# sp-uhh/buddy

Measured on AMD Instinct MI355X. Metric: diffusion steps/sec (4 s@16 kHz utterance, blind Euler-Heun DPS, order 1, 10 operator updates/step), higher is better.
Workload: dtype f32 (GEMM operands -- Winograd-domain and 1x1 / NIN -- as two-term f16 splits, 2^-22, fp32 accumulation)

## Files before the change

buddy_amd/_lib.py:

```python
from __future__ import annotations

import ctypes as C
import os

_HERE = os.path.dirname(os.path.abspath(__file__))
LIB_PATH = os.path.join(_HERE, "libbuddy_hip.so")


class BuddyHipError(RuntimeError):
    pass


_lib = None

_f32p = C.c_void_p
_SIGS = {
    "buddy_last_error": (C.c_char_p, []),
    "buddy_version": (C.c_int, []),
    "buddy_ncsnpp_param_count": (C.c_int, [C.c_int, C.POINTER(C.c_int), C.c_int, C.c_int, C.POINTER(C.c_longlong)]),
    "buddy_ncsnpp_create": (C.c_int, [_f32p, C.c_longlong, C.c_int, C.POINTER(C.c_int), C.c_int, C.c_int, C.c_int, C.c_int,
                                      C.POINTER(C.c_void_p)]),
    "buddy_ncsnpp_param_count_attn": (C.c_int, [C.c_int, C.POINTER(C.c_int), C.c_int, C.c_int, C.c_int, C.POINTER(C.c_longlong)]),
    "buddy_ncsnpp_create_attn": (C.c_int, [_f32p, C.c_longlong, C.c_int, C.POINTER(C.c_int), C.c_int, C.c_int, C.c_int, C.c_int, C.c_int,
                                           C.POINTER(C.c_void_p)]),
# ... 116 lines not shown
    "buddy_blindop_degrade": (C.c_int, [C.c_void_p, _f32p, _f32p, C.c_void_p]),
    "buddy_blindop_time_rir": (C.c_int, [C.c_void_p, _f32p, C.c_void_p]),
    "buddy_blindop_design_filter": (C.c_int, [C.c_void_p, _f32p, C.c_void_p]),
    "buddy_blindop_apply_stft": (C.c_int, [C.c_void_p, _f32p, _f32p, C.c_void_p]),
    "buddy_blindop_degrade_vjp": (C.c_int, [C.c_void_p, _f32p, _f32p, _f32p, _f32p, C.c_void_p]),
    "buddy_blindop_time_rir_vjp": (C.c_int, [C.c_void_p, _f32p, _f32p, C.c_void_p]),
    "buddy_blindop_update_H_vjp": (C.c_int, [C.c_void_p, _f32p, _f32p, _f32p, _f32p, C.c_void_p]),
    "buddy_blindop_stft": (C.c_int, [C.c_void_p, _f32p, C.c_int, _f32p, C.c_void_p]),
    "buddy_blindop_stft_adjoint": (C.c_int, [C.c_void_p, _f32p, C.c_int, _f32p, C.c_void_p]),
    "buddy_blindop_stft_loss": (C.c_int, [C.c_void_p, _f32p, _f32p, C.c_int, C.c_float, _f32p, _f32p, _f32p, C.c_void_p]),
    "buddy_blindop_set_compression": (C.c_int, [C.c_void_p, C.c_float]),
    "buddy_blindop_set_loss_norm": (C.c_int, [C.c_void_p, C.c_int]),
    "buddy_blindop_set_loss": (C.c_int, [C.c_void_p, C.c_int, C.c_int, C.c_int, C.c_float]),
    "buddy_blindop_set_freq_weights": (C.c_int, [C.c_void_p, C.c_int, _f32p]),
    "buddy_blindop_lengths": (C.c_int, [C.c_void_p, C.POINTER(C.c_int), C.POINTER(C.c_int), C.POINTER(C.c_int), C.POINTER(C.c_int)]),
    "buddy_blindop_minphase": (C.c_int, [C.c_void_p, _f32p, _f32p, C.c_void_p]),
    "buddy_blindop_project": (C.c_int, [C.c_void_p, C.c_void_p]),
    "buddy_blindop_get_adam": (C.c_int, [C.c_void_p, _f32p, _f32p, _f32p, _f32p, _f32p, _f32p, C.POINTER(C.c_int), C.c_void_p]),
    "buddy_blindop_rec_loss_grad": (C.c_int, [C.c_void_p, _f32p, C.c_float, _f32p, _f32p, C.c_void_p]),
    "buddy_blindop_fir_loss_grad": (C.c_int, [C.c_void_p, _f32p, _f32p, C.c_longlong, C.c_int, C.c_float, _f32p, _f32p, C.c_void_p]),
    "buddy_blindop_param_grads": (C.c_int, [C.c_void_p, _f32p, _f32p, C.c_float, C.c_float, C.c_float, _f32p, _f32p, _f32p, _f32p, C.c_void_p]),
    "buddy_blindop_optimize": (C.c_int, [C.c_void_p, _f32p, _f32p, C.c_float, C.c_int, C.c_float, C.c_float, C.c_float, C.c_float, C.c_float,
                                         C.c_float, C.c_void_p]),
    "buddy_fir": (C.c_int, [_f32p, _f32p, C.c_longlong, _f32p, C.c_int, C.c_int, C.c_int, C.c_int, C.c_void_p]),
}
EXPORTED = sorted(_SIGS)


def load():
    global _lib
# ... 43 lines not shown
```

buddy_amd/csrc/capi.hip:

```cpp
#include "../../include/buddy_hip.h"
#include "common.h"
#include "net.h"

#include <cstring>

using namespace buddy;

namespace buddy {
void launch_axpby_rows(const float* x, const float* y, const float* a, const float* c, float* out, int B, int L, hipStream_t st);
void launch_row_moments(const float* x, double* out, int B, int L, hipStream_t st);
void launch_perturb(const float* x, const float* eps, float scale, float* out, long long n, hipStream_t st);
void launch_dps_update(const float* x_hat, const float* x_den, const float* lh, const float* lh_scale_b, const float* den_scale_b, const float* base, const float* d_prev,
                       float t, float dt, float w_prev, float w_cur, float* out, float* d_out, float* x_den_out, int B, int L, hipStream_t st);
void launch_row_scale(const float* x, float* out, int B, int L, int mode, float p0, float p1, hipStream_t st);
void launch_fill_rows4(float* out, int B, float v0, float v1, float v2, float v3, hipStream_t st);
void launch_mfma_ubench(const float* seed, float* out, int blocks, int iters, unsigned long long* clk, hipStream_t st);
void launch_mfma_ubench_bf16(const float* seed, float* out, int blocks, int iters, unsigned long long* clk, hipStream_t st);
int launch_hbm_ubench(const void* src, void* dst, long long bytes, int mode, int nt, int blocks, hipStream_t st);
void launch_fir(const float* x, const float* h, long long h_stride, float* y, int B, int L, int M, int adjoint, hipStream_t st);
}

static int finish() {
  hipError_t e = hipGetLastError();
  if (e != hipSuccess) { set_error(std::string("kernel launch: ") + hipGetErrorString(e)); return BUDDY_ERR_HIP; }
// ... 658 lines not shown
int buddy_blindop_time_rir_vjp(void* h, const float* g_rir, float* g_H, void* stream) { BOP_CHECK(h); if (!g_rir || !g_H) { set_error("null"); return BUDDY_ERR_ARG; } return blindop_time_rir_vjp((BlindOp*)h, g_rir, g_H, (hipStream_t)stream); }
int buddy_blindop_update_H_vjp(void* h, const float* g_H, float* g_decay, float* g_weights, float* g_phases, void* stream) {
  BOP_CHECK(h); if (!g_H) { set_error("null"); return BUDDY_ERR_ARG; } return blindop_update_H_vjp((BlindOp*)h, g_H, g_decay, g_weights, g_phases, (hipStream_t)stream);
}
int buddy_blindop_stft(void* h, const float* x, int len, float* X, void* stream) { BOP_CHECK(h); if (!x || !X) { set_error("null"); return BUDDY_ERR_ARG; } return blindop_stft_len((BlindOp*)h, x, len, X, (hipStream_t)stream); }
int buddy_blindop_stft_adjoint(void* h, const float* G, int len, float* g_x, void* stream) { BOP_CHECK(h); if (!G || !g_x) { set_error("null"); return BUDDY_ERR_ARG; } return blindop_stft_len_adj((BlindOp*)h, G, len, g_x, (hipStream_t)stream); }
int buddy_blindop_stft_loss(void* h, const float* a, const float* b, int len, float weight, float* loss, float* g_a, float* g_b, void* stream) {
  BOP_CHECK(h); if (!a || !b || !loss) { set_error("null"); return BUDDY_ERR_ARG; } return blindop_stft_loss((BlindOp*)h, a, b, len, weight, loss, g_a, g_b, (hipStream_t)stream);
}
int buddy_blindop_set_compression(void* h, float comp) { BOP_CHECK(h); return blindop_set_compression((BlindOp*)h, comp); }
int buddy_blindop_set_loss_norm(void* h, int mode) { BOP_CHECK(h); return blindop_set_loss_norm((BlindOp*)h, mode); }
int buddy_blindop_set_loss(void* h, int slot, int kind, int freq_weighting, float compression) {
  BOP_CHECK(h); return blindop_set_loss((BlindOp*)h, slot, kind, freq_weighting, compression);
}
int buddy_blindop_set_freq_weights(void* h, int freq_weighting, const float* w) { BOP_CHECK(h); return blindop_set_freq_weights((BlindOp*)h, freq_weighting, w); }
int buddy_blindop_lengths(void* h, int* L, int* Lr, int* T, int* Td) { BOP_CHECK(h); return blindop_lengths((BlindOp*)h, L, Lr, T, Td); }
int buddy_blindop_minphase(void* h, const float* hin, float* out, void* stream) { BOP_CHECK(h); if (!hin || !out) { set_error("null"); return BUDDY_ERR_ARG; } return blindop_minphase((BlindOp*)h, hin, out, (hipStream_t)stream); }
int buddy_blindop_project(void* h, void* stream) { BOP_CHECK(h); return blindop_project((BlindOp*)h, (hipStream_t)stream); }
int buddy_blindop_get_adam(void* h, float* m_decay, float* v_decay, float* m_weights, float* v_weights, float* m_phases, float* v_phases, int* step,
                           void* stream) {
  BOP_CHECK(h); return blindop_get_adam((BlindOp*)h, m_decay, v_decay, m_weights, v_weights, m_phases, v_phases, step, (hipStream_t)stream);
}
int buddy_blindop_rec_loss_grad(void* h, const float* x_den, float weight, float* loss, float* g_x, void* stream) {
  BOP_CHECK(h); if (!x_den || !loss) { set_error("null"); return BUDDY_ERR_ARG; }
  return blindop_rec_loss_grad((BlindOp*)h, x_den, weight, loss, g_x, (hipStream_t)stream);
}
int buddy_blindop_fir_loss_grad(void* h, const float* x_den, const float* rir, long long rir_stride, int M, float weight, float* loss, float* g_x,
                                void* stream) {
  BOP_CHECK(h); if (!x_den || !rir || !loss || M < 1) { set_error("bad arguments"); return BUDDY_ERR_ARG; }
  return blindop_fir_loss_grad((BlindOp*)h, x_den, rir, rir_stride, M, weight, loss, g_x, (hipStream_t)stream);
// ... 14 lines not shown
```

buddy_amd/csrc/net.h:

```cpp
#pragma once
#include <hip/hip_runtime.h>
#include <string>

namespace buddy {

struct NetCfg { int nf; int ch_mult[8]; int nlev; int nrb; int n_fft; int hop; int attn_mask; };
struct Net;

void set_error(const std::string& s);
const char* last_error();
long long param_count(const NetCfg& c);
int net_create(const float* host_params, long long n, const NetCfg& cfg, Net** out);
void net_destroy(Net* N);
int net_replica(Net* src, Net** out);
int net_weight_bytes(Net* N, long long* params, long long* packed, long long* lazy, int* lazy_forms);
int net_set_option(Net* N, const char* key, int value);
int net_get_option(Net* N, const char* key, int* value);
int net_set_gemm(Net* N, int mode);
int net_set_attention(Net* N, int mode);
int net_set_fir(Net* N, int fir);
int net_reserve(Net* N, int B, int L, int with_vjp, long long* bytes);
int net_forward(Net* N, const float* x, const float* cnoise, const float* cin_b, const float* cskip_b, const float* cout_b, float* y, int B, int L,
                int save, hipStream_t st);
int net_vjp(Net* N, const float* cot, float* gx, hipStream_t st);
// ... 23 lines not shown
int blindop_apply_stft(BlindOp* o, const float* x, float* X_ref, hipStream_t st);
int blindop_minphase(BlindOp* o, const float* h, float* out, hipStream_t st);
int blindop_project(BlindOp* o, hipStream_t st);
int blindop_get_adam(BlindOp* o, float* m_decay, float* v_decay, float* m_wts, float* v_wts, float* m_phases, float* v_phases, int* step, hipStream_t st);
int blindop_degrade_vjp(BlindOp* o, const float* x, const float* g_y, float* g_x, float* g_H_ref, hipStream_t st);
int blindop_time_rir_vjp(BlindOp* o, const float* g_rir, float* g_H_ref, hipStream_t st);
int blindop_update_H_vjp(BlindOp* o, const float* g_H_ref, float* g_decay, float* g_wts, float* g_phases_ref, hipStream_t st);
int blindop_stft_len(BlindOp* o, const float* x, int len, float* X_ref, hipStream_t st);
int blindop_stft_len_adj(BlindOp* o, const float* G_ref, int len, float* g_x, hipStream_t st);
int blindop_stft_loss(BlindOp* o, const float* a, const float* b, int len, float weight, float* loss, float* g_a, float* g_b, hipStream_t st);
int blindop_set_compression(BlindOp* o, float comp);
int blindop_set_loss_norm(BlindOp* o, int mode);
int blindop_set_loss(BlindOp* o, int slot, int kind, int freq_weighting, float comp);
int blindop_set_freq_weights(BlindOp* o, int freq_weighting, const float* w);
int blindop_lengths(BlindOp* o, int* L, int* Lr, int* T, int* Td);
int blindop_rec_loss_grad(BlindOp* o, const float* x_den, float weight, float* loss, float* g_x, hipStream_t st);
int blindop_fir_loss_grad(BlindOp* o, const float* x_den, const float* rir, long long rir_stride, int M, float weight, float* loss, float* g_x,
                          hipStream_t st);
int blindop_param_grads(BlindOp* o, const float* x_den, const float* noise, float t_op, float w_rec, float w_reg, float* g_decay, float* g_wts,
                        float* g_phases_ref, float* losses, hipStream_t st);
int blindop_optimize(BlindOp* o, const float* x_den, const float* noise, float t_op, int n_iters, float w_rec, float w_reg, float lr, float b1,
                     float b2, float wd, hipStream_t st);

}
```

buddy_amd/csrc/operator.hip:

```cpp
#include "common.h"
#include "net.h"

#include <cmath>
#include <cstring>
#include <vector>

namespace buddy {

#define HIPCHK(x) do { hipError_t e_ = (x); if (e_ != hipSuccess) { set_error(std::string(#x) + ": " + hipGetErrorString(e_)); return BUDDY_ERR_HIP; } } while (0)

namespace {
constexpr int FB = 513, LDSP = 1028, NFFT = 1024, WIN = 512, HOP = 128;
constexpr int N2 = 25856, F1 = 101, F2 = 256;
constexpr double PI = 3.14159265358979323846;

constexpr int FT = 4;
__global__ __launch_bounds__(256) void fir_kernel_sb(const float* X, long long xs, const float* H, float* Y, int U, int T, int Nf) {
  const int TG = (T + FT - 1) / FT;
  const long long total = (long long)U * TG * FB;
  for (long long i = (long long)blockIdx.x * 256 + threadIdx.x; i < total; i += (long long)gridDim.x * 256) {
    const int f = (int)(i % FB); const int t0 = (int)((i / FB) % TG) * FT; const int u = (int)(i / ((long long)FB * TG));
    const float2* Xu = reinterpret_cast<const float2*>(X + (long long)u * xs) + f;
    const float2* Hu = reinterpret_cast<const float2*>(H + (long long)u * Nf * LDSP) + f;
    auto ldx = [&](int tt) { return (tt >= 0 && tt < T) ? Xu[(long long)tt * (LDSP / 2)] : make_float2(0.f, 0.f); };
// ... 202 lines not shown
}

__device__ __forceinline__ float2 compress(float2 x, float p) {
  const float r = sqrtf(x.x * x.x + x.y * x.y);
  if (r == 0.f) return make_float2(powf(1e-8f, p), 0.f);
  const float rho = powf(r + 1e-8f, p) / r;
  return make_float2(x.x * rho, x.y * rho);
}
__global__ __launch_bounds__(256) void compress_kernel(const float* X, float* Xc, long long rows, float p) {
  const long long total = rows * FB;
  for (long long i = (long long)blockIdx.x * 256 + threadIdx.x; i < total; i += (long long)gridDim.x * 256) {
    const long long r = i / FB; const int f = (int)(i % FB);
    reinterpret_cast<float2*>(Xc + r * LDSP)[f] = compress(reinterpret_cast<const float2*>(X + r * LDSP)[f], p);
  }
}
struct LossJob { const float* Rc; const float* Xh; float* G; double* partial; int T; float kappa; int blocks; };
struct LossJobs { LossJob j[2]; };
__global__ __launch_bounds__(256) void comp_loss_kernel(LossJobs jobs, float p) {
  __shared__ double red[256];
  const bool second = (int)blockIdx.x >= jobs.j[0].blocks;
  const LossJob& jb = jobs.j[second ? 1 : 0];
  const float* Rc = jb.Rc; const float* Xh = jb.Xh; float* G = jb.G;
  const int T = jb.T, nblk = jb.blocks, bx = (int)blockIdx.x - (second ? jobs.j[0].blocks : 0);
  const float kappa = jb.kappa;
  const int u = blockIdx.y;
  const long long total = (long long)T * FB;
  double acc = 0.0;
  for (long long i = (long long)bx * 256 + threadIdx.x; i < total; i += (long long)nblk * 256) {
    const long long t = i / FB; const int f = (int)(i % FB);
    const long long row = ((long long)u * T + t) * LDSP;
    const float2 x = reinterpret_cast<const float2*>(Xh + row)[f];
    const float2 rc = Rc ? reinterpret_cast<const float2*>(Rc + row)[f] : compress(reinterpret_cast<const float2*>(G + row)[f], p);
    const float r = sqrtf(x.x * x.x + x.y * x.y);
    float2 g = make_float2(0.f, 0.f);
    float2 xc;
    if (r == 0.f) {
      xc = make_float2(powf(1e-8f, p), 0.f);
    } else {
      const float ir = 1.f / r, re = r + 1e-8f;
      const float cr = x.x * ir, ci = x.y * ir;
      const float rho = powf(re, p);
      xc = make_float2(rho * cr, rho * ci);
      const float dr = xc.x - rc.x, di = xc.y - rc.y;
      const float a = dr * cr + di * ci;
      const float b = dr * ci - di * cr;
      const float gr = 2.f * kappa * a * p * (rho / re);
      const float gt = -2.f * kappa * rho * b * ir;
      g = make_float2(gr * cr - gt * ci, gr * ci + gt * cr);
    }
    const float dr = xc.x - rc.x, di = xc.y - rc.y;
    acc += (double)(dr * dr + di * di);
    if (G) reinterpret_cast<float2*>(G + row)[f] = g;
  }
  red[threadIdx.x] = acc;
  __syncthreads();
  for (int off = 128; off > 0; off >>= 1) { if (threadIdx.x < off) red[threadIdx.x] += red[threadIdx.x + off]; __syncthreads(); }
  if (threadIdx.x == 0) jb.partial[(long long)u * nblk + bx] = red[0];
}
__global__ void loss_finalize_kernel(const double* partial, int nblk, float kappa, float* loss, int accumulate) {
  const int u = blockIdx.x;
  if (threadIdx.x != 0) return;
  double s = 0.0;
  for (int i = 0; i < nblk; ++i) s += partial[(long long)u * nblk + i];
  const float v = (float)(s * (double)kappa);
  loss[u] = accumulate ? loss[u] + v : v;
}
// ... 614 lines not shown
  const bool ok = row < (second ? jobs.j[1].rows : jobs.j[0].rows);
  const float2* f = reinterpret_cast<const float2*>(in + (ok ? row : 0) * LDSP);
  float2 v[16];
#pragma unroll
  for (int a = 0; a < 16; ++a) {
    const int k = 64 * a + r;
    float2 x = make_float2(0.f, 0.f);
    if (ok && k <= 512) { x = f[k]; if (cf && k != 0 && k != 512) { x.x *= 2.f; x.y *= 2.f; } }
    v[a] = x;
  }
  fft1024_core<1>(v, S[w], tw, r);
  if (!ok) return;
#pragma unroll
  for (int c1 = 0; c1 < 8; ++c1) { const int n = r + 64 * c1; frames[row * WIN + n] = fac * win[n] * v[c1].x; }
}

__global__ __launch_bounds__(256) void adam_kernel(float* p, const float* g, float* m, float* v, long long n, float lr, float b1, float b2, float eps,
                                                   float wd, float bc1, float bc2_sqrt, const int* step_dev, const float2* bc_tab) {
  if (step_dev) { const float2 bc = bc_tab[*step_dev]; bc1 = bc.x; bc2_sqrt = bc.y; }
  for (long long i = (long long)blockIdx.x * 256 + threadIdx.x; i < n; i += (long long)gridDim.x * 256) {
    float gi = g[i];
    if (wd != 0.f) gi += wd * p[i];
    const float mi = m[i] + (gi - m[i]) * (1.f - b1);
    const float vi = v[i] * b2 + (1.f - b2) * gi * gi;
    m[i] = mi; v[i] = vi;
    const float denom = sqrtf(vi) / bc2_sqrt + eps;
    p[i] = p[i] - (lr / bc1) * (mi / denom);
  }
}
__global__ void set_scalar_kernel(float* dst, float v) { *dst = v; }
// ... 120 lines not shown
struct BlindOp {
  BlindOpCfg c;
  int U = 0, L = 0, T = 0, Td = 0, Lr = 0, Lh = 0, Lm = 0, E = 0, NB = 0, K = 0, Nf = 0;
  hipStream_t st = nullptr;
  std::vector<void*> allocs;
  float *ones = nullptr, *env_T = nullptr, *env_d = nullptr, *env_c = nullptr;
  float norm = 1.f;
  int *idx = nullptr, *fge = nullptr; float *frac = nullptr, *corr = nullptr, *dpm = nullptr;
  float2 *w101 = nullptr, *w256 = nullptr, *twN = nullptr, *w1024r = nullptr, *w64t = nullptr; float* win = nullptr;
  float *decay = nullptr, *wts = nullptr, *phi = nullptr;
  float *m_d = nullptr, *v_d = nullptr, *m_w = nullptr, *v_w = nullptr, *m_p = nullptr, *v_p = nullptr;
  int adam_step = 0;
  static constexpr int MAXSTEP = 65536;
  int* d_step = nullptr; float* d_scal = nullptr; float2* bc_tab = nullptr; float tab_b1 = -1.f, tab_b2 = -1.f;
  float *xden_buf = nullptr, *noise_buf = nullptr; int noise_iters = 0;
  hipStream_t cap_stream = nullptr; hipGraphExec_t gexec = nullptr; int g_iters = -1; float g_hp[7] = {0, 0, 0, 0, 0, 0, 0};
  float *H = nullptr, *Yc = nullptr, *Xdelta = nullptr;
  float *frames = nullptr, *X1 = nullptr, *X2 = nullptr, *X3 = nullptr, *Ybuf = nullptr, *sig1 = nullptr, *sig2 = nullptr;
  float *frames_b = nullptr, *X2_b = nullptr, *X3_b = nullptr, *Ybuf_b = nullptr; double* partial_b = nullptr;
  struct LossDesc { int kind; int fw; float comp; };
  static constexpr int NSLOT = 4, NFW = 5;
  LossDesc slot[NSLOT] = {{0, 0, 0.667f}, {0, 0, 0.667f}, {0, 0, 0.667f}, {0, 0, 0.667f}};
  float* wtab = nullptr; unsigned wtab_set = 1u;
  float *Ytd = nullptr, *Yc1 = nullptr;
  bool fused_loop = false;
  bool big_lds = false;
  float *A = nullptr, *Apre = nullptr, *logdm = nullptr, *dmv = nullptr, *gdm = nullptr, *Fin = nullptr, *GFin = nullptr, *GH = nullptr;
  float *gphi = nullptr, *gdecay = nullptr, *gw = nullptr, *hm = nullptr, *gh0 = nullptr;
  float2 *c1 = nullptr, *c2 = nullptr, *Hf = nullptr;
  float *Mabs = nullptr, *phim = nullptr, *gM = nullptr;
  double* partial = nullptr; float* losses = nullptr;
// ... 129 lines not shown
  static bool is_comp(const LossDesc& d) { return d.kind <= LK_COMP_MEAN; }
  static bool legacy(const LossDesc& d) { return is_comp(d) && d.fw == 0; }
  static bool same_target(const LossDesc& a, const LossDesc& b) {
    if (is_td(a) || is_td(b)) return is_td(a) && is_td(b);
    if (!is_spec(a) || !is_spec(b) || a.fw != b.fw) return false;
    if (is_comp(a) || is_comp(b)) return is_comp(a) && is_comp(b) && a.comp == b.comp;
    return a.kind == b.kind;
  }
  const float* wrow(const LossDesc& d) const { return d.fw ? wtab + (size_t)d.fw * FB : nullptr; }
  const float* target(int s) const { return is_td(slot[s]) ? Ytd : (s == 1 && !same_target(slot[0], slot[1]) ? Yc1 : Yc); }
  void spec_target(int s, const float* X, float* R, long long rows) {
    const LossDesc& d = slot[s];
    if (legacy(d)) hipLaunchKernelGGL(compress_kernel, dim3(gridf(rows * FB)), dim3(256), 0, st, X, R, rows, d.comp);
    else hipLaunchKernelGGL(spec_target_kernel, dim3(gridf(rows * FB)), dim3(256), 0, st, X, R, rows, d.kind, wrow(d), d.comp);
  }
  static constexpr int LOSS_BLK = 64, LOSS_BLK_B = 32;
  void comp_loss2(int s0, const float* Rc0, const float* Xh0, float* G0, int T0, float w0, float* out0, int s1, const float* Rc1, const float* Xh1, float* G1,
                  int T1, float w1, float* out1, bool two) {
    const LossDesc& d0 = slot[s0];
    const LossDesc& d1 = slot[two ? s1 : s0];
    auto kap = [&](const LossDesc& d, float w, int Tn) { return d.kind == LK_COMP_SUMMEAN ? w / (float)Tn : (d.kind == LK_COMP_MEAN ? w / ((float)Tn * (float)FB) : w); };
    const float k0 = kap(d0, w0, T0), k1 = two ? kap(d1, w1, T1) : 0.f;
    const unsigned grid = LOSS_BLK + (two ? LOSS_BLK_B : 0);
    if (legacy(d0) && (!two || (legacy(d1) && d1.comp == d0.comp))) {
      LossJobs jobs; std::memset(&jobs, 0, sizeof(jobs));
      jobs.j[0] = LossJob{Rc0, Xh0, G0, partial, T0, k0, LOSS_BLK};
      if (two) jobs.j[1] = LossJob{Rc1, Xh1, G1, partial_b, T1, k1, LOSS_BLK_B};
      hipLaunchKernelGGL(comp_loss_kernel, dim3(grid, U), dim3(256), 0, st, jobs, d0.comp);
    } else {
      SpecJobs jobs; std::memset(&jobs, 0, sizeof(jobs));
      jobs.j[0] = SpecJob{Rc0, Xh0, G0, partial, wrow(d0), T0, k0, d0.comp, d0.kind, LOSS_BLK};
      if (two) jobs.j[1] = SpecJob{Rc1, Xh1, G1, partial_b, wrow(d1), T1, k1, d1.comp, d1.kind, LOSS_BLK_B};
      hipLaunchKernelGGL(spec_loss_kernel, dim3(grid, U), dim3(256), 0, st, jobs);
    }
    if (!fused_loop) {
      hipLaunchKernelGGL(loss_finalize_kernel, dim3(U), dim3(32), 0, st, (const double*)partial, LOSS_BLK, k0, out0, 0);
      if (two) hipLaunchKernelGGL(loss_finalize_kernel, dim3(U), dim3(32), 0, st, (const double*)partial_b, LOSS_BLK_B, k1, out1, 0);
    }
  }
  void comp_loss(int s, const float* Rcx, const float* Xh, float* G, int Tn, float weight, float* out) {
    comp_loss2(s, Rcx, Xh, G, Tn, weight, out, s, nullptr, nullptr, nullptr, 0, 0.f, nullptr, false);
  }
  void td_loss(int s, const float* y, const float* yh, float* g, int len, float weight, float* out, double* part, const float* noise = nullptr,
               float t = 0.f, const float* t_dev = nullptr) {
    const float k = slot[s].kind == LK_L2_MEAN ? weight / (float)len : weight;
    const TdJob jb{y, yh, g, part, noise, t_dev, t, len, k, LOSS_BLK};
    hipLaunchKernelGGL(td_loss_kernel, dim3(LOSS_BLK, U), dim3(256), 0, st, jb);
    if (!fused_loop) hipLaunchKernelGGL(loss_finalize_kernel, dim3(U), dim3(32), 0, st, (const double*)part, LOSS_BLK, k, out, 0);
  }
  void reg_chain(const float* noise, float t_op, const float* t_op_dev, float w_reg) {
    const int Q = WIN + WIN / 2;
    if (is_td(slot[2])) {
      time_rir(rir);
      td_loss(2, nullptr, rir, sig2, Lr, w_reg, losses + U, partial_b, noise, t_op, t_op_dev);
      istft_adj(sig2, Td, Q, env_d, Lr, norm, X2);
      return;
// ... 81 lines not shown
  const int T = o->T > Td ? o->T : Td;
  const int Lmax = L > o->Lr ? L : o->Lr;
  const size_t specT = (size_t)U_ * T * LDSP + 8, specH = (size_t)U_ * (Nf + 2) * LDSP + 8;
  DA(decay, U_ * o->E * o->NB); DA(wts, U_ * o->E * o->NB); DA(phi, (size_t)U_ * Nf * FB);
  DA(m_d, U_ * o->E * o->NB); DA(v_d, U_ * o->E * o->NB); DA(m_w, U_ * o->E * o->NB); DA(v_w, U_ * o->E * o->NB);
  DA(m_p, (size_t)U_ * Nf * FB); DA(v_p, (size_t)U_ * Nf * FB);
  DA(H, specH); DA(Yc, specT); DA(Xdelta, (size_t)Td * LDSP + 8);
  DA(frames, (size_t)U_ * (T + 2) * WIN);
  DA(X1, specT); DA(X2, specT); DA(X3, specT); DA(Ybuf, specT); DA(sig1, (size_t)U_ * (Lmax + 8)); DA(sig2, (size_t)U_ * (Lmax + 8));
  DA(A, (size_t)U_ * Nf * FB); DA(Apre, (size_t)U_ * Nf * FB); DA(logdm, U_ * Nf * o->K); DA(dmv, U_ * Nf * o->K); DA(gdm, U_ * Nf * o->K);
  DA(Fin, specH); DA(GFin, specH); DA(GH, specH); DA(gphi, (size_t)U_ * Nf * FB);
  DA(gdecay, U_ * o->E * o->NB); DA(gw, U_ * o->E * o->NB);
  DA(hm, (size_t)U_ * o->Lm); DA(gh0, (size_t)U_ * o->Lh);
  DA(c1, (size_t)U_ * N2); DA(c2, (size_t)U_ * N2); DA(Hf, (size_t)U_ * N2);
  DA(Mabs, (size_t)U_ * N2); DA(phim, (size_t)U_ * N2); DA(gM, (size_t)U_ * N2);
  DA(partial, (size_t)U_ * 64); DA(losses, (size_t)U_ * 4);
  o->big_lds = hipFuncSetAttribute((const void*)fir_sb_lds_kernel<FIR_NF>, hipFuncAttributeMaxDynamicSharedMemorySize, 96 * 1024) == hipSuccess;
  {
    const size_t specD = (size_t)U_ * Td * LDSP + 8;
    DA(frames_b, (size_t)U_ * (Td + 2) * WIN);
    DA(X2_b, specD); DA(X3_b, specD); DA(Ybuf_b, specD); DA(partial_b, (size_t)U_ * 64);
  }
  DA(rir, (size_t)U_ * o->Lr); DA(Rc, (size_t)U_ * Td * LDSP + 8);
  DA(dpm, (size_t)Nf * FB);
  DA(d_step, 4); DA(d_scal, 4); DA(bc_tab, BlindOp::MAXSTEP); DA(xden_buf, (size_t)U_ * L);
  {
    const int saveU = o->U; o->U = 1; o->st = nullptr;
    std::vector<float> imp((size_t)o->Lr, 0.f);
    imp[0] = (float)(WIN / (HOP * 2.0));
    float* tmp_sig = o->rir;
    HIPCHK(hipMemcpy(tmp_sig, imp.data(), (size_t)o->Lh * 4, hipMemcpyHostToDevice));
    o->stft(tmp_sig, o->Lh, WIN - HOP, Nf, 1.f, o->GH);
    HIPCHK(hipDeviceSynchronize());
    std::vector<float> hs((size_t)Nf * LDSP);
    HIPCHK(hipMemcpy(hs.data(), o->GH, hs.size() * 4, hipMemcpyDeviceToHost));
    std::vector<float> dpm((size_t)Nf * FB);
// ... 231 lines not shown
  if (fw != 0 && !((o->wtab_set >> fw) & 1u)) { set_error("frequency weighting: its table has not been uploaded (buddy_blindop_set_freq_weights)"); return BUDDY_ERR_ARG; }
  if (BlindOp::is_comp(d) && !(comp > 0.f && comp <= 1.f)) { set_error("compression factor must be in (0, 1]"); return BUDDY_ERR_ARG; }
  BlindOp::LossDesc nd = d;
  if (!BlindOp::is_comp(d)) nd.comp = o->slot[s].comp;
  BlindOp::LossDesc next[2] = {o->slot[0], o->slot[1]};
  if (s < 2) next[s] = nd;
  if ((BlindOp::is_td(next[0]) || BlindOp::is_td(next[1])) && !o->Ytd && o->dalloc(&o->Ytd, (size_t)o->U * o->L)) { set_error("hipMalloc failed"); return BUDDY_ERR_HIP; }
  if (BlindOp::is_spec(next[1]) && !BlindOp::same_target(next[0], next[1]) && !o->Yc1 && o->dalloc(&o->Yc1, (size_t)o->U * o->T * LDSP + 8)) {
    set_error("hipMalloc failed"); return BUDDY_ERR_HIP;
  }
  const BlindOp::LossDesc& od = o->slot[s];
  if ((od.kind != nd.kind || od.fw != nd.fw || od.comp != nd.comp) && s < 3 && o->gexec) { (void)hipGraphExecDestroy(o->gexec); o->gexec = nullptr; }
  o->slot[s] = nd;
  return BUDDY_OK;
}
int blindop_lengths(BlindOp* o, int* L, int* Lr, int* T, int* Td) { if (L) *L = o->L; if (Lr) *Lr = o->Lr; if (T) *T = o->T; if (Td) *Td = o->Td; return BUDDY_OK; }

int blindop_rec_loss_grad(BlindOp* o, const float* x_den, float weight, float* loss, float* g_x, hipStream_t st) {
  o->st = st;
  const int U = o->U, T = o->T, L = o->L;
  o->stft(x_den, L, WIN, T, 1.f / o->norm, o->X1);
  o->fir(o->X1, (long long)T * LDSP, T, o->Ybuf);
  if (BlindOp::is_td(o->slot[0])) {
    o->istft(o->Ybuf, T, WIN + WIN / 2, o->env_T, L, o->norm, o->sig1);
    o->td_loss(0, o->Ytd, o->sig1, g_x ? o->sig2 : nullptr, L, weight, loss, o->partial);
    if (g_x) o->istft_adj(o->sig2, T, WIN + WIN / 2, o->env_T, L, o->norm, o->X2);
  } else {
    o->istft_stft(o->Ybuf, T, WIN + WIN / 2, o->env_T, L, o->norm, WIN, T, 1.f / o->norm, o->X2);
    o->comp_loss(0, o->target(0), o->X2, g_x ? o->X3 : nullptr, T, weight, loss);
    if (g_x) o->stft_adj_istft_adj(o->X3, L, WIN, T, 1.f / o->norm, T, WIN + WIN / 2, o->env_T, o->norm, o->X2);
// ... 24 lines not shown
  return BUDDY_OK;
}

static int param_grads(BlindOp* o, const float* x_den, const float* noise, float t_op, float w_rec, float w_reg, bool have_Xd, const float* t_op_dev = nullptr) {
  const int U = o->U, T = o->T, Td = o->Td, L = o->L, Nf = o->Nf;
  hipStream_t st = o->st;
  const float norm = o->norm;
  o->update_H();
  if (!have_Xd) o->stft(x_den, L, WIN, T, 1.f / norm, o->X1);
  const bool rec_on = o->slot[1].kind != LK_NONE;
  if (noise && o->fir_lds_ok() && BlindOp::is_spec(o->slot[1]) && BlindOp::is_spec(o->slot[2])) {
    const int Q = WIN + WIN / 2;
    o->fir2(o->X1, (long long)T * LDSP, T, o->Ybuf, o->Xdelta, 0LL, Td, o->Ybuf_b);
    o->c2r2(o->Ybuf, (long long)U * T, o->frames, o->Ybuf_b, (long long)U * Td, o->frames_b, norm / NFFT, 1);
    {
      const BlindOp::R2cReq rq[3] = {
          {R2cSrc{nullptr, o->frames, L, WIN, T, Q, o->env_T, nullptr, nullptr, 0.f, nullptr}, T, o->X2},
          {R2cSrc{nullptr, o->frames_b, o->Lr, WIN, Td, Q, o->env_d, nullptr, nullptr, 0.f, nullptr}, Td, o->X2_b},
          {R2cSrc{nullptr, o->frames_b, o->Lr, WIN, Td, Q, o->env_d, nullptr, noise, t_op, t_op_dev}, Td, o->X3_b}};
      o->r2c_multi(rq, 3, 1.f / norm, 0);
    }
    o->comp_loss2(1, o->target(1), o->X2, o->X3, T, w_rec, o->losses, 2, nullptr, o->X2_b, o->X3_b, Td, w_reg, o->losses + U, true);
    o->c2r2(o->X3, (long long)U * T, o->frames, o->X3_b, (long long)U * Td, o->frames_b, 1.f / norm, 0);
    {
      const BlindOp::R2cReq rq[2] = {
          {R2cSrc{nullptr, o->frames, L, Q, T, WIN, o->ones, o->env_T, nullptr, 0.f, nullptr}, T, o->X2},
          {R2cSrc{nullptr, o->frames_b, o->Lr, Q, Td, WIN, o->ones, o->env_d, nullptr, 0.f, nullptr}, Td, o->X2_b}};
      o->r2c_multi(rq, 2, norm / NFFT, 1);
    }
    o->gradh2(o->X1, (long long)T * LDSP, o->X2, T, o->Xdelta, 0LL, o->X2_b, Td, 0);
  } else {
    if (BlindOp::is_td(o->slot[1])) {
      o->fir(o->X1, (long long)T * LDSP, T, o->Ybuf);
      o->istft(o->Ybuf, T, WIN + WIN / 2, o->env_T, L, norm, o->sig1);
      o->td_loss(1, o->Ytd, o->sig1, o->sig2, L, w_rec, o->losses, o->partial);
      o->istft_adj(o->sig2, T, WIN + WIN / 2, o->env_T, L, norm, o->X2);
      o->gradh(o->X1, (long long)T * LDSP, o->X2, T, 0);
    } else if (rec_on) {
      o->fir(o->X1, (long long)T * LDSP, T, o->Ybuf);
      o->istft_stft(o->Ybuf, T, WIN + WIN / 2, o->env_T, L, norm, WIN, T, 1.f / norm, o->X2);
      o->comp_loss(1, o->target(1), o->X2, o->X3, T, w_rec, o->losses);
      o->stft_adj_istft_adj(o->X3, L, WIN, T, 1.f / norm, T, WIN + WIN / 2, o->env_T, norm, o->X2);
// ... 84 lines not shown
  if (!o->gexec || o->g_iters != n_iters || std::memcmp(hp, o->g_hp, sizeof(hp)) != 0) {
    if (o->gexec) { (void)hipGraphExecDestroy(o->gexec); o->gexec = nullptr; }
    if (!o->cap_stream) HIPCHK(hipStreamCreateWithFlags(&o->cap_stream, hipStreamNonBlocking));
    const bool prof = igemm_prof_enabled();
    igemm_prof_enable(0);
    const int step0 = o->adam_step;
    HIPCHK(hipStreamBeginCapture(o->cap_stream, hipStreamCaptureModeThreadLocal));
    o->st = o->cap_stream;
    for (int it = 0; it < n_iters; ++it)
      optimize_iteration(o, o->xden_buf, noise ? o->noise_buf + (long long)it * U * o->Lr : nullptr, t_op, w_rec, w_reg, lr, b1, b2, wd, it > 0, true);
    hipGraph_t graph = nullptr;
    const hipError_t ce = hipStreamEndCapture(o->cap_stream, &graph);
    o->st = st; o->adam_step = step0;
    igemm_prof_enable(prof ? 1 : 0);
    if (ce != hipSuccess || !graph) { set_error(std::string("optimize_op graph capture failed: ") + hipGetErrorString(ce)); return BUDDY_ERR_HIP; }
    const hipError_t ie = hipGraphInstantiate(&o->gexec, graph, nullptr, nullptr, 0);
    (void)hipGraphDestroy(graph);
    if (ie != hipSuccess) { o->gexec = nullptr; set_error(std::string("hipGraphInstantiate failed: ") + hipGetErrorString(ie)); return BUDDY_ERR_HIP; }
    o->g_iters = n_iters; std::memcpy(o->g_hp, hp, sizeof(hp));
  }
  HIPCHK(hipGraphLaunch(o->gexec, st));
  o->adam_step += n_iters;
  return BUDDY_OK;
}

}
```

include/buddy_hip.h:

```cpp
#ifndef BUDDY_HIP_H
#define BUDDY_HIP_H
#ifdef __cplusplus
extern "C" {
#endif

const char* buddy_last_error(void);
int buddy_version(void);


int buddy_ncsnpp_param_count(int nf, const int* ch_mult, int n_levels, int num_res_blocks, long long* count);

int buddy_ncsnpp_create(const float* host_params, long long n_params, int nf, const int* ch_mult, int n_levels,
                        int num_res_blocks, int n_fft, int hop, void** handle);
int buddy_ncsnpp_param_count_attn(int nf, const int* ch_mult, int n_levels, int num_res_blocks, int attn_mask, long long* count);
int buddy_ncsnpp_create_attn(const float* host_params, long long n_params, int nf, const int* ch_mult, int n_levels,
                             int num_res_blocks, int n_fft, int hop, int attn_mask, void** handle);
int buddy_ncsnpp_destroy(void* handle);
int buddy_ncsnpp_replica(void* handle, void** replica);
int buddy_ncsnpp_weight_bytes(void* handle, long long* params, long long* packed, long long* lazy, int* lazy_forms);
int buddy_conv3_weight_prep(const float* w_oihw, int O, int I, int dgrad, int kind, float* out, void* stream);

int buddy_ncsnpp_reserve(void* handle, int B, int L, int with_vjp, long long* bytes);

int buddy_ncsnpp_forward(void* handle, const float* x, const float* cnoise, const float* cin, const float* cskip,
// ... 147 lines not shown
int buddy_blindop_time_rir(void* handle, float* rir , void* stream);
int buddy_blindop_design_filter(void* handle, float* A, void* stream);
int buddy_blindop_apply_stft(void* handle, const float* x, float* X, void* stream);
int buddy_blindop_minphase(void* handle, const float* h, float* out, void* stream);
int buddy_blindop_degrade_vjp(void* handle, const float* x, const float* g_y, float* g_x, float* g_H, void* stream);
int buddy_blindop_time_rir_vjp(void* handle, const float* g_rir , float* g_H, void* stream);
int buddy_blindop_update_H_vjp(void* handle, const float* g_H, float* g_decay, float* g_weights, float* g_phases, void* stream);
int buddy_blindop_stft(void* handle, const float* x, int len, float* X, void* stream);
int buddy_blindop_stft_adjoint(void* handle, const float* G, int len, float* g_x, void* stream);
int buddy_blindop_stft_loss(void* handle, const float* a, const float* b, int len, float weight, float* loss, float* g_a, float* g_b, void* stream);
int buddy_blindop_set_compression(void* handle, float compression_factor);
int buddy_blindop_set_loss_norm(void* handle, int mode);
int buddy_blindop_set_loss(void* handle, int slot, int kind, int freq_weighting, float compression);
int buddy_blindop_set_freq_weights(void* handle, int freq_weighting, const float* w);
int buddy_blindop_lengths(void* handle, int* L, int* L_rir, int* frames, int* frames_rir);
int buddy_blindop_project(void* handle, void* stream);
int buddy_blindop_get_adam(void* handle, float* m_decay, float* v_decay, float* m_weights, float* v_weights, float* m_phases, float* v_phases,
                           int* step , void* stream);
int buddy_blindop_rec_loss_grad(void* handle, const float* x_den, float weight, float* loss, float* g_x, void* stream);
int buddy_blindop_fir_loss_grad(void* handle, const float* x_den, const float* rir, long long rir_stride, int M, float weight, float* loss,
                                float* g_x, void* stream);
int buddy_blindop_param_grads(void* handle, const float* x_den, const float* noise, float t_op, float w_rec, float w_reg, float* g_decay,
                              float* g_weights, float* g_phases, float* losses, void* stream);
int buddy_blindop_optimize(void* handle, const float* x_den, const float* noise, float t_op, int n_iters, float w_rec, float w_reg, float lr,
                           float beta1, float beta2, float weight_decay, void* stream);

#ifdef __cplusplus
}
#endif
#endif
// ... 1 lines not shown
```

Baseline: 143.3.

## Fuse STFT, spectral loss gradient and inverse STFT into one sandwich kernel

```diff
diff --git a/buddy_amd/_lib.py b/buddy_amd/_lib.py
--- a/buddy_amd/_lib.py
+++ b/buddy_amd/_lib.py
@@ -154,6 +154,7 @@
     "buddy_blindop_set_loss": (C.c_int, [C.c_void_p, C.c_int, C.c_int, C.c_int, C.c_float]),
     "buddy_blindop_set_freq_weights": (C.c_int, [C.c_void_p, C.c_int, _f32p]),
     "buddy_blindop_lengths": (C.c_int, [C.c_void_p, C.POINTER(C.c_int), C.POINTER(C.c_int), C.POINTER(C.c_int), C.POINTER(C.c_int)]),
+    "buddy_blindop_graph_kernel_nodes": (C.c_int, [C.c_void_p, C.POINTER(C.c_int), C.POINTER(C.c_int)]),
     "buddy_blindop_minphase": (C.c_int, [C.c_void_p, _f32p, _f32p, C.c_void_p]),
     "buddy_blindop_project": (C.c_int, [C.c_void_p, C.c_void_p]),
     "buddy_blindop_get_adam": (C.c_int, [C.c_void_p, _f32p, _f32p, _f32p, _f32p, _f32p, _f32p, C.POINTER(C.c_int), C.c_void_p]),
diff --git a/buddy_amd/csrc/capi.hip b/buddy_amd/csrc/capi.hip
--- a/buddy_amd/csrc/capi.hip
+++ b/buddy_amd/csrc/capi.hip
@@ -696,6 +696,7 @@
   BOP_CHECK(h); return blindop_set_loss((BlindOp*)h, slot, kind, freq_weighting, compression);
 }
 int buddy_blindop_set_freq_weights(void* h, int freq_weighting, const float* w) { BOP_CHECK(h); return blindop_set_freq_weights((BlindOp*)h, freq_weighting, w); }
+int buddy_blindop_graph_kernel_nodes(void* h, int* nodes, int* iters) { BOP_CHECK(h); return blindop_graph_kernel_nodes((BlindOp*)h, nodes, iters); }
 int buddy_blindop_lengths(void* h, int* L, int* Lr, int* T, int* Td) { BOP_CHECK(h); return blindop_lengths((BlindOp*)h, L, Lr, T, Td); }
 int buddy_blindop_minphase(void* h, const float* hin, float* out, void* stream) { BOP_CHECK(h); if (!hin || !out) { set_error("null"); return BUDDY_ERR_ARG; } return blindop_minphase((BlindOp*)h, hin, out, (hipStream_t)stream); }
 int buddy_blindop_project(void* h, void* stream) { BOP_CHECK(h); return blindop_project((BlindOp*)h, (hipStream_t)stream); }
diff --git a/buddy_amd/csrc/net.h b/buddy_amd/csrc/net.h
--- a/buddy_amd/csrc/net.h
+++ b/buddy_amd/csrc/net.h
@@ -61,6 +61,7 @@
 int blindop_set_loss(BlindOp* o, int slot, int kind, int freq_weighting, float comp);
 int blindop_set_freq_weights(BlindOp* o, int freq_weighting, const float* w);
 int blindop_lengths(BlindOp* o, int* L, int* Lr, int* T, int* Td);
+int blindop_graph_kernel_nodes(BlindOp* o, int* nodes, int* iters);
 int blindop_rec_loss_grad(BlindOp* o, const float* x_den, float weight, float* loss, float* g_x, hipStream_t st);
 int blindop_fir_loss_grad(BlindOp* o, const float* x_den, const float* rir, long long rir_stride, int M, float weight, float* loss, float* g_x,
                           hipStream_t st);
diff --git a/buddy_amd/csrc/operator.hip b/buddy_amd/csrc/operator.hip
--- a/buddy_amd/csrc/operator.hip
+++ b/buddy_amd/csrc/operator.hip
@@ -240,6 +240,27 @@
     reinterpret_cast<float2*>(Xc + r * LDSP)[f] = compress(reinterpret_cast<const float2*>(X + r * LDSP)[f], p);
   }
 }
+__device__ __forceinline__ float comp_loss_bin(float2 x, float2 rc, float kappa, float p, float2& g) {
+  const float r = sqrtf(x.x * x.x + x.y * x.y);
+  g = make_float2(0.f, 0.f);
+  float2 xc;
+  if (r == 0.f) {
+    xc = make_float2(powf(1e-8f, p), 0.f);
+  } else {
+    const float ir = 1.f / r, re = r + 1e-8f;
+    const float cr = x.x * ir, ci = x.y * ir;
+    const float rho = powf(re, p);
+    xc = make_float2(rho * cr, rho * ci);
+    const float dr = xc.x - rc.x, di = xc.y - rc.y;
+    const float a = dr * cr + di * ci;
+    const float b = dr * ci - di * cr;
+    const float gr = 2.f * kappa * a * p * (rho / re);
+    const float gt = -2.f * kappa * rho * b * ir;
+    g = make_float2(gr * cr - gt * ci, gr * ci + gt * cr);
+  }
+  const float dr = xc.x - rc.x, di = xc.y - rc.y;
+  return dr * dr + di * di;
+}
 struct LossJob { const float* Rc; const float* Xh; float* G; double* partial; int T; float kappa; int blocks; };
 struct LossJobs { LossJob j[2]; };
 __global__ __launch_bounds__(256) void comp_loss_kernel(LossJobs jobs, float p) {
@@ -257,25 +278,8 @@
     const long long row = ((long long)u * T + t) * LDSP;
     const float2 x = reinterpret_cast<const float2*>(Xh + row)[f];
     const float2 rc = Rc ? reinterpret_cast<const float2*>(Rc + row)[f] : compress(reinterpret_cast<const float2*>(G + row)[f], p);
-    const float r = sqrtf(x.x * x.x + x.y * x.y);
-    float2 g = make_float2(0.f, 0.f);
-    float2 xc;
-    if (r == 0.f) {
-      xc = make_float2(powf(1e-8f, p), 0.f);
-    } else {
-      const float ir = 1.f / r, re = r + 1e-8f;
-      const float cr = x.x * ir, ci = x.y * ir;
-      const float rho = powf(re, p);
-      xc = make_float2(rho * cr, rho * ci);
-      const float dr = xc.x - rc.x, di = xc.y - rc.y;
-      const float a = dr * cr + di * ci;
-      const float b = dr * ci - di * cr;
-      const float gr = 2.f * kappa * a * p * (rho / re);
-      const float gt = -2.f * kappa * rho * b * ir;
-      g = make_float2(gr * cr - gt * ci, gr * ci + gt * cr);
-    }
-    const float dr = xc.x - rc.x, di = xc.y - rc.y;
-    acc += (double)(dr * dr + di * di);
+    float2 g;
+    acc += (double)comp_loss_bin(x, rc, kappa, p, g);
     if (G) reinterpret_cast<float2*>(G + row)[f] = g;
   }
   red[threadIdx.x] = acc;
@@ -920,6 +924,107 @@
 #pragma unroll
   for (int c1 = 0; c1 < 8; ++c1) { const int n = r + 64 * c1; frames[row * WIN + n] = fac * win[n] * v[c1].x; }
 }
+struct SwJob { R2cSrc sc; int Tn; int rows; int blocks; const float* R; float* out; double* partial; const float* w; float kappa; float p; int kind; };
+struct SwJobs { SwJob j[2]; };
+template <int K> __device__ __forceinline__ float sw_spec_bin(float2 x, float2 tg, bool have_R, const float* w, int f, float kappa, float p, float2& g) {
+  const float wf = w ? w[f] : 1.f;
+  float2 rc = tg;
+  if (!have_R) { if (w) { tg.x *= wf; tg.y *= wf; } rc = spec_phi<K>(tg, p); }
+  if (w) { x.x *= wf; x.y *= wf; }
+  const float2 ph = spec_phi<K>(x, p);
+  const float dr = ph.x - rc.x, di = ph.y - rc.y;
+  const float2 gg = spec_grad<K>(x, dr, di, p);
+  const float s = kappa * wf;
+  g = make_float2(s * gg.x, s * gg.y);
+  return dr * dr + di * di;
+}
+__device__ __forceinline__ float sw_bin(int kind, float2 x, float2 tg, bool have_R, const float* w, int f, float kappa, float p, float2& g) {
+  switch (kind) {
+    case LK_STFT_SUM: return sw_spec_bin<LK_STFT_SUM>(x, tg, have_R, w, f, kappa, p, g);
+    case LK_STFT_MAG_SUM: return sw_spec_bin<LK_STFT_MAG_SUM>(x, tg, have_R, w, f, kappa, p, g);
+    case LK_STFT_LOGMAG_SUM: return sw_spec_bin<LK_STFT_LOGMAG_SUM>(x, tg, have_R, w, f, kappa, p, g);
+    case LK_LOG_STFT_SUM: return sw_spec_bin<LK_LOG_STFT_SUM>(x, tg, have_R, w, f, kappa, p, g);
+    case LK_COMP_SUMMEAN: case LK_COMP_SUM: case LK_COMP_MEAN: return sw_spec_bin<LK_COMP_SUMMEAN>(x, tg, have_R, w, f, kappa, p, g);
+    default: return comp_loss_bin(x, have_R ? tg : compress(tg, p), kappa, p, g);
+  }
+}
+__global__ __launch_bounds__(256) void spec_sandwich_kernel(SwJobs jobs, const float* __restrict__ win, const float2* __restrict__ Wrow,
+                                                            const float2* __restrict__ W64t, float fac_f, float fac_i) {
+  __shared__ float2 S[4][16 * FLD];
+  const int w = threadIdx.x >> 6, r = threadIdx.x & 63;
+  const bool second = (int)blockIdx.x >= jobs.j[0].blocks;
+  const SwJob& jb = jobs.j[second ? 1 : 0];
+  const R2cSrc& sc = jb.sc;
+  const long long row = (long long)((int)blockIdx.x - (second ? jobs.j[0].blocks : 0)) * 4 + w;
+  if (row >= jb.rows) return;
+  Fft1024Tw tw; fft1024_load_tw(tw, Wrow, W64t, r);
+  const int Tn = jb.Tn;
+  const int u = (int)(row / Tn), t = (int)(row % Tn);
+  const bool have_R = jb.R != nullptr;
+  const float add_scale = have_R ? 0.f : (sc.add_scale_dev ? *sc.add_scale_dev : sc.add_scale);
+  float2 v[16], vt[16];
+#pragma unroll
+  for (int a = 0; a < 16; ++a) { v[a] = make_float2(0.f, 0.f); vt[a] = make_float2(0.f, 0.f); }
+  {
+    float fv[8][4], ea[8], ad[8];
+    bool in[8], fin[8][4];
+    const long long ubase = (long long)u * sc.Ls;
+#pragma unroll
+    for (int a = 0; a < 8; ++a) {
+      const int n = 64 * a + r, s = HOP * t + n - sc.P;
+      in[a] = s >= 0 && s < sc.Ls;
+      const int sc_s = in[a] ? s : 0;
+      const int j = sc_s + sc.Q, tq = j >> 7, m0 = j & (HOP - 1);
+#pragma unroll
+      for (int k = 0; k < 4; ++k) {
+        const int tt = tq - 3 + k;
+        fin[a][k] = tt >= 0 && tt < sc.Tsrc;
+        fv[a][k] = sc.fr[((long long)u * sc.Tsrc + (fin[a][k] ? tt : 0)) * WIN + m0 + HOP * (3 - k)];
+      }
+      ea[a] = sc.envA[j];
+      ad[a] = (!have_R && sc.add) ? sc.add[ubase + sc_s] : 0.f;
+    }
+#pragma unroll
+    for (int a = 0; a < 8; ++a) {
+      float val = 0.f;
+#pragma unroll
+      for (int k = 0; k < 4; ++k) val += fin[a][k] ? fv[a][k] : 0.f;
+      val *= ea[a];
+      const float wn = win[64 * a + r];
+      v[a].x = (in[a] ? val : 0.f) * wn;
+      if (!have_R) { float vn = val; vn += add_scale * ad[a]; vt[a].x = (in[a] ? vn : 0.f) * wn; }
+    }
+  }
+  fft1024_core<-1>(v, S[w], tw, r);
+  if (!have_R) { wave_lds_sync(); fft1024_core<-1>(vt, S[w], tw, r); }
+  const float2* Rrow = reinterpret_cast<const float2*>(jb.R + (have_R ? row * LDSP : 0));
+  float2 tg[9];
+#pragma unroll
+  for (int c1 = 0; c1 < 8; ++c1) tg[c1] = have_R ? Rrow[r + 64 * c1] : make_float2(vt[c1].x * fac_f, vt[c1].y * fac_f);
+  tg[8] = have_R ? Rrow[512] : make_float2(vt[8].x * fac_f, vt[8].y * fac_f);
+  double acc = 0.0;
+#pragma unroll
+  for (int c1 = 0; c1 < 8; ++c1) {
+    float2 g;
+    acc += (double)sw_bin(jb.kind, make_float2(v[c1].x * fac_f, v[c1].y * fac_f), tg[c1], have_R, jb.w, r + 64 * c1, jb.kappa, jb.p, g);
+    v[c1] = g;
+  }
+  {
+    float2 g;
+    const float d2 = sw_bin(jb.kind, make_float2(v[8].x * fac_f, v[8].y * fac_f), tg[8], have_R, jb.w, 512, jb.kappa, jb.p, g);
+    if (r == 0) acc += (double)d2;
+    v[8] = r == 0 ? g : make_float2(0.f, 0.f);
+  }
+#pragma unroll
+  for (int a = 9; a < 16; ++a) v[a] = make_float2(0.f, 0.f);
+#pragma unroll
+  for (int off = 32; off > 0; off >>= 1) acc += __shfl_xor(acc, off, 64);
+  if (r == 0) jb.partial[row] = acc;
+  wave_lds_sync();
+  fft1024_core<1>(v, S[w], tw, r);
+#pragma unroll
+  for (int c1 = 0; c1 < 8; ++c1) { const int n = r + 64 * c1; jb.out[row * WIN + n] = fac_i * win[n] * v[c1].x; }
+}
 
 __global__ __launch_bounds__(256) void adam_kernel(float* p, const float* g, float* m, float* v, long long n, float lr, float b1, float b2, float eps,
                                                    float wd, float bc1, float bc2_sqrt, const int* step_dev, const float2* bc_tab) {
@@ -1070,7 +1175,7 @@
   static constexpr int MAXSTEP = 65536;
   int* d_step = nullptr; float* d_scal = nullptr; float2* bc_tab = nullptr; float tab_b1 = -1.f, tab_b2 = -1.f;
   float *xden_buf = nullptr, *noise_buf = nullptr; int noise_iters = 0;
-  hipStream_t cap_stream = nullptr; hipGraphExec_t gexec = nullptr; int g_iters = -1; float g_hp[7] = {0, 0, 0, 0, 0, 0, 0};
+  hipStream_t cap_stream = nullptr; hipGraphExec_t gexec = nullptr; int g_iters = -1, g_knodes = 0; float g_hp[7] = {0, 0, 0, 0, 0, 0, 0};
   float *H = nullptr, *Yc = nullptr, *Xdelta = nullptr;
   float *frames = nullptr, *X1 = nullptr, *X2 = nullptr, *X3 = nullptr, *Ybuf = nullptr, *sig1 = nullptr, *sig2 = nullptr;
   float *frames_b = nullptr, *X2_b = nullptr, *X3_b = nullptr, *Ybuf_b = nullptr; double* partial_b = nullptr;
@@ -1230,32 +1335,43 @@
     if (legacy(d)) hipLaunchKernelGGL(compress_kernel, dim3(gridf(rows * FB)), dim3(256), 0, st, X, R, rows, d.comp);
     else hipLaunchKernelGGL(spec_target_kernel, dim3(gridf(rows * FB)), dim3(256), 0, st, X, R, rows, d.kind, wrow(d), d.comp);
   }
-  static constexpr int LOSS_BLK = 64, LOSS_BLK_B = 32;
-  void comp_loss2(int s0, const float* Rc0, const float* Xh0, float* G0, int T0, float w0, float* out0, int s1, const float* Rc1, const float* Xh1, float* G1,
-                  int T1, float w1, float* out1, bool two) {
-    const LossDesc& d0 = slot[s0];
-    const LossDesc& d1 = slot[two ? s1 : s0];
-    auto kap = [&](const LossDesc& d, float w, int Tn) { return d.kind == LK_COMP_SUMMEAN ? w / (float)Tn : (d.kind == LK_COMP_MEAN ? w / ((float)Tn * (float)FB) : w); };
-    const float k0 = kap(d0, w0, T0), k1 = two ? kap(d1, w1, T1) : 0.f;
-    const unsigned grid = LOSS_BLK + (two ? LOSS_BLK_B : 0);
-    if (legacy(d0) && (!two || (legacy(d1) && d1.comp == d0.comp))) {
+  static constexpr int LOSS_BLK = 64;
+  static float kap(const LossDesc& d, float w, int Tn) { return d.kind == LK_COMP_SUMMEAN ? w / (float)Tn : (d.kind == LK_COMP_MEAN ? w / ((float)Tn * (float)FB) : w); }
+  void comp_loss(int s, const float* Rcx, const float* Xh, float* G, int Tn, float weight, float* out) {
+    const LossDesc& d = slot[s];
+    const float k = kap(d, weight, Tn);
+    if (legacy(d)) {
       LossJobs jobs; std::memset(&jobs, 0, sizeof(jobs));
-      jobs.j[0] = LossJob{Rc0, Xh0, G0, partial, T0, k0, LOSS_BLK};
-      if (two) jobs.j[1] = LossJob{Rc1, Xh1, G1, partial_b, T1, k1, LOSS_BLK_B};
-      hipLaunchKernelGGL(comp_loss_kernel, dim3(grid, U), dim3(256), 0, st, jobs, d0.comp);
+      jobs.j[0] = LossJob{Rcx, Xh, G, partial, Tn, k, LOSS_BLK};
+      hipLaunchKernelGGL(comp_loss_kernel, dim3(LOSS_BLK, U), dim3(256), 0, st, jobs, d.comp);
     } else {
       SpecJobs jobs; std::memset(&jobs, 0, sizeof(jobs));
-      jobs.j[0] = SpecJob{Rc0, Xh0, G0, partial, wrow(d0), T0, k0, d0.comp, d0.kind, LOSS_BLK};
-      if (two) jobs.j[1] = SpecJob{Rc1, Xh1, G1, partial_b, wrow(d1), T1, k1, d1.comp, d1.kind, LOSS_BLK_B};
-      hipLaunchKernelGGL(spec_loss_kernel, dim3(grid, U), dim3(256), 0, st, jobs);
-    }
-    if (!fused_loop) {
-      hipLaunchKernelGGL(loss_finalize_kernel, dim3(U), dim3(32), 0, st, (const double*)partial, LOSS_BLK, k0, out0, 0);
-      if (two) hipLaunchKernelGGL(loss_finalize_kernel, dim3(U), dim3(32), 0, st, (const double*)partial_b, LOSS_BLK_B, k1, out1, 0);
-    }
-  }
-  void comp_loss(int s, const float* Rcx, const float* Xh, float* G, int Tn, float weight, float* out) {
-    comp_loss2(s, Rcx, Xh, G, Tn, weight, out, s, nullptr, nullptr, nullptr, 0, 0.f, nullptr, false);
+      jobs.j[0] = SpecJob{Rcx, Xh, G, partial, wrow(d), Tn, k, d.comp, d.kind, LOSS_BLK};
+      hipLaunchKernelGGL(spec_loss_kernel, dim3(LOSS_BLK, U), dim3(256), 0, st, jobs);
+    }
+    if (!fused_loop)
+      hipLaunchKernelGGL(loss_finalize_kernel, dim3(U), dim3(32), 0, st, (const double*)partial, LOSS_BLK, k, out, 0);
+  }
+  struct SwTerm { int s; const float* fr; int Ls; int Tn; const float* env; const float* R; const float* noise; float* out; float w; float* loss; double* part; };
+  void spec_sandwich(const SwTerm& a, const SwTerm& b, float t_op, const float* t_op_dev) {
+    const int Q = WIN + WIN / 2;
+    SwJobs jobs; std::memset(&jobs, 0, sizeof(jobs));
+    const SwTerm* tm[2] = {&a, &b};
+    const bool leg = legacy(slot[a.s]) && legacy(slot[b.s]) && slot[a.s].comp == slot[b.s].comp;
+    float k[2];
+    for (int i = 0; i < 2; ++i) {
+      const SwTerm& q = *tm[i];
+      const LossDesc& d = slot[q.s];
+      k[i] = kap(d, q.w, q.Tn);
+      SwJob& j = jobs.j[i];
+      j.sc = R2cSrc{nullptr, q.fr, q.Ls, WIN, q.Tn, Q, q.env, nullptr, q.noise, t_op, t_op_dev};
+      j.Tn = q.Tn; j.rows = U * q.Tn; j.blocks = (U * q.Tn + 3) / 4; j.R = q.R; j.out = q.out; j.partial = q.part;
+      j.w = leg ? nullptr : wrow(d); j.kappa = k[i]; j.p = d.comp; j.kind = leg ? -1 : d.kind;
+    }
+    hipLaunchKernelGGL(spec_sandwich_kernel, dim3((unsigned)(jobs.j[0].blocks + jobs.j[1].blocks)), dim3(256), 0, st, jobs, (const float*)win, (const float2*)w1024r,
+                       (const float2*)w64t, 1.f / norm, 1.f / norm);
+    if (!fused_loop)
+      for (int i = 0; i < 2; ++i) hipLaunchKernelGGL(loss_finalize_kernel, dim3(U), dim3(32), 0, st, (const double*)tm[i]->part, tm[i]->Tn, k[i], tm[i]->loss, 0);
   }
   void td_loss(int s, const float* y, const float* yh, float* g, int len, float weight, float* out, double* part, const float* noise = nullptr,
                float t = 0.f, const float* t_dev = nullptr) {
@@ -1367,12 +1483,12 @@
   DA(hm, (size_t)U_ * o->Lm); DA(gh0, (size_t)U_ * o->Lh);
   DA(c1, (size_t)U_ * N2); DA(c2, (size_t)U_ * N2); DA(Hf, (size_t)U_ * N2);
   DA(Mabs, (size_t)U_ * N2); DA(phim, (size_t)U_ * N2); DA(gM, (size_t)U_ * N2);
-  DA(partial, (size_t)U_ * 64); DA(losses, (size_t)U_ * 4);
+  DA(partial, (size_t)U_ * (T > 64 ? T : 64)); DA(losses, (size_t)U_ * 4);
   o->big_lds = hipFuncSetAttribute((const void*)fir_sb_lds_kernel<FIR_NF>, hipFuncAttributeMaxDynamicSharedMemorySize, 96 * 1024) == hipSuccess;
   {
     const size_t specD = (size_t)U_ * Td * LDSP + 8;
     DA(frames_b, (size_t)U_ * (Td + 2) * WIN);
-    DA(X2_b, specD); DA(X3_b, specD); DA(Ybuf_b, specD); DA(partial_b, (size_t)U_ * 64);
+    DA(X2_b, specD); DA(X3_b, specD); DA(Ybuf_b, specD); DA(partial_b, (size_t)U_ * (Td > 64 ? Td : 64));
   }
   DA(rir, (size_t)U_ * o->Lr); DA(Rc, (size_t)U_ * Td * LDSP + 8);
   DA(dpm, (size_t)Nf * FB);
@@ -1634,6 +1750,11 @@
   o->slot[s] = nd;
   return BUDDY_OK;
 }
+int blindop_graph_kernel_nodes(BlindOp* o, int* nodes, int* iters) {
+  if (nodes) *nodes = o->gexec ? o->g_knodes : 0;
+  if (iters) *iters = o->gexec ? o->g_iters : 0;
+  return BUDDY_OK;
+}
 int blindop_lengths(BlindOp* o, int* L, int* Lr, int* T, int* Td) { if (L) *L = o->L; if (Lr) *Lr = o->Lr; if (T) *T = o->T; if (Td) *Td = o->Td; return BUDDY_OK; }
 
 int blindop_rec_loss_grad(BlindOp* o, const float* x_den, float weight, float* loss, float* g_x, hipStream_t st) {
@@ -1688,18 +1809,14 @@
     o->fir2(o->X1, (long long)T * LDSP, T, o->Ybuf, o->Xdelta, 0LL, Td, o->Ybuf_b);
     o->c2r2(o->Ybuf, (long long)U * T, o->frames, o->Ybuf_b, (long long)U * Td, o->frames_b, norm / NFFT, 1);
     {
-      const BlindOp::R2cReq rq[3] = {
-          {R2cSrc{nullptr, o->frames, L, WIN, T, Q, o->env_T, nullptr, nullptr, 0.f, nullptr}, T, o->X2},
-          {R2cSrc{nullptr, o->frames_b, o->Lr, WIN, Td, Q, o->env_d, nullptr, nullptr, 0.f, nullptr}, Td, o->X2_b},
-          {R2cSrc{nullptr, o->frames_b, o->Lr, WIN, Td, Q, o->env_d, nullptr, noise, t_op, t_op_dev}, Td, o->X3_b}};
-      o->r2c_multi(rq, 3, 1.f / norm, 0);
-    }
-    o->comp_loss2(1, o->target(1), o->X2, o->X3, T, w_rec, o->losses, 2, nullptr, o->X2_b, o->X3_b, Td, w_reg, o->losses + U, true);
-    o->c2r2(o->X3, (long long)U * T, o->frames, o->X3_b, (long long)U * Td, o->frames_b, 1.f / norm, 0);
+      const BlindOp::SwTerm ta{1, o->frames, L, T, o->env_T, o->target(1), nullptr, o->X3, w_rec, o->losses, o->partial};
+      const BlindOp::SwTerm tb{2, o->frames_b, o->Lr, Td, o->env_d, nullptr, noise, o->X3_b, w_reg, o->losses + U, o->partial_b};
+      o->spec_sandwich(ta, tb, t_op, t_op_dev);
+    }
     {
       const BlindOp::R2cReq rq[2] = {
-          {R2cSrc{nullptr, o->frames, L, Q, T, WIN, o->ones, o->env_T, nullptr, 0.f, nullptr}, T, o->X2},
-          {R2cSrc{nullptr, o->frames_b, o->Lr, Q, Td, WIN, o->ones, o->env_d, nullptr, 0.f, nullptr}, Td, o->X2_b}};
+          {R2cSrc{nullptr, o->X3, L, Q, T, WIN, o->ones, o->env_T, nullptr, 0.f, nullptr}, T, o->X2},
+          {R2cSrc{nullptr, o->X3_b, o->Lr, Q, Td, WIN, o->ones, o->env_d, nullptr, 0.f, nullptr}, Td, o->X2_b}};
       o->r2c_multi(rq, 2, norm / NFFT, 1);
     }
     o->gradh2(o->X1, (long long)T * LDSP, o->X2, T, o->Xdelta, 0LL, o->X2_b, Td, 0);
@@ -1814,6 +1931,15 @@
     o->st = st; o->adam_step = step0;
     igemm_prof_enable(prof ? 1 : 0);
     if (ce != hipSuccess || !graph) { set_error(std::string("optimize_op graph capture failed: ") + hipGetErrorString(ce)); return BUDDY_ERR_HIP; }
+    {
+      size_t nn = 0;
+      o->g_knodes = 0;
+      if (hipGraphGetNodes(graph, nullptr, &nn) == hipSuccess && nn) {
+        std::vector<hipGraphNode_t> nd(nn);
+        if (hipGraphGetNodes(graph, nd.data(), &nn) == hipSuccess)
+          for (size_t i = 0; i < nn; ++i) { hipGraphNodeType ty; if (hipGraphNodeGetType(nd[i], &ty) == hipSuccess && ty == hipGraphNodeTypeKernel) o->g_knodes += 1; }
+      }
+    }
     const hipError_t ie = hipGraphInstantiate(&o->gexec, graph, nullptr, nullptr, 0);
     (void)hipGraphDestroy(graph);
     if (ie != hipSuccess) { o->gexec = nullptr; set_error(std::string("hipGraphInstantiate failed: ") + hipGetErrorString(ie)); return BUDDY_ERR_HIP; }
diff --git a/include/buddy_hip.h b/include/buddy_hip.h
--- a/include/buddy_hip.h
+++ b/include/buddy_hip.h
@@ -185,6 +185,7 @@
 int buddy_blindop_set_loss(void* handle, int slot, int kind, int freq_weighting, float compression);
 int buddy_blindop_set_freq_weights(void* handle, int freq_weighting, const float* w);
 int buddy_blindop_lengths(void* handle, int* L, int* L_rir, int* frames, int* frames_rir);
+int buddy_blindop_graph_kernel_nodes(void* handle, int* nodes, int* iters);
 int buddy_blindop_project(void* handle, void* stream);
 int buddy_blindop_get_adam(void* handle, float* m_decay, float* v_decay, float* m_weights, float* v_weights, float* m_phases, float* v_phases,
                            int* step , void* stream);
```

Result: no change. 143.3, median of 3 (+0.0%).
